# kohnakagawa/md_neighbor_list

Measured on AMD Instinct MI355X. Metric: Verlet-list build ms and Mpairs/s at N=1M rho=1.0; achieved HBM GB/s, higher is better.
Workload: dtype f32

## Files before the change

### md_neighbor_list_amd/csrc/nl_api.hip

```cpp
#include "../../include/nl_hip.h"

#include <hip/hip_runtime.h>

#include <algorithm>
#include <cmath>
#include <cstdio>
#include <cstdlib>
#include <cstring>
#include <new>
#include <tuple>
#include <type_traits>
#include <vector>

#include "nl_devbuf.hpp"
#include "nl_kernels.hpp"
#include "nl_stage.hpp"

using namespace nl;

namespace {

struct HostResult {
  uint32_t status;
  uint32_t tickets[17];
// ... 24 lines not shown
  auto tie() const { return std::tie(q, stride, gid, n_rows, n, n_ghost_lo, z_lo, mzl, slab, dyn, dyn_host, n_est); }
  bool operator==(const BuildArgs& o) const { return tie() == o.tie(); }
};

enum Binning : int32_t {
  BINNING_BUCKET,
  BINNING_TWO_PASS,
  BINNING_ATOMIC,
};
enum Search : int32_t {
  SEARCH_ROWS,
  SEARCH_MASKS,
  SEARCH_DENSE,
  SEARCH_SWEEPS,
};

struct BuildPlan {
  int32_t binning = BINNING_ATOMIC;
  int32_t cap_row = 0;
  bool split = false;
  int32_t search = SEARCH_SWEEPS;
  int32_t rows_v = 0;
  int32_t mask_nb = 1;
  bool small = false;
  bool rows12 = false;
  bool list = true;
  bool full = false;
  bool wide = false;
  bool filter = false;
  bool images = false;
  int32_t pbc = 0;
  int32_t idc = 0;
  int32_t id_shift = 0;
  bool id_rows = false;
  Box box = {{0, 0, 0}, 0, 0, 0};
  int32_t tilt = 0;
  auto tie() const {
    return std::tie(binning, cap_row, split, search, rows_v, mask_nb, small, rows12, list, full, wide, filter, images, pbc, idc, id_shift, id_rows,
                    box.L[0], box.L[1], box.L[2], box.xy, box.xz, box.yz, tilt);
  }
  bool operator==(const BuildPlan& o) const { return tie() == o.tie(); }
};

struct GraphKey {
  BuildArgs args;
  BuildPlan plan;
  int64_t capacity = 0;
  uint64_t buffers_epoch = 0;
  uint64_t ex_gen = 0;
  uint64_t ty_gen = 0;
  int32_t update = 0;
  double skin = 0;
  auto tie() const { return std::tie(args, plan, capacity, buffers_epoch, ex_gen, ty_gen, update, skin); }
  bool operator==(const GraphKey& o) const { return tie() == o.tie(); }
};

}

struct nl_handle_s {
  int dtype = NL_F32, device = 0;
  double rc = 0, L[3] = {0, 0, 0}, rc2 = 0;
  int32_t m[3] = {0, 0, 0};
  int64_t ncell = 0;
  double xy = 0, xz = 0, yz = 0, shear[3] = {0, 0, 0}, L0[3] = {0, 0, 0};
  int64_t mesh_cells_cap = 0, mesh_rows_cap = 0;
  DevBuf<double> lat_dev;
  float ims_f[3];
  double ims_d[3];
  float rc2_f = 0;
  float ms_f[3];

// ... 10 lines not shown
  DevBuf<int32_t> sorted_gid;
  DevBuf<int32_t> count;
  DevBuf<void> key_pointer;
  DevBuf<void> kp_alt;
  bool kp_alt_valid = false;
  int offset_width = 0;
  DevBuf<int32_t> progress;
  int32_t* row_count = nullptr;
  DevBuf<int32_t> row_start;
  DevBuf<int32_t> blk_base;
  DevBuf<void> tmp_pos;
  DevBuf<int32_t> tmp_row;
  size_t tmp_slots = 0;
  DevBuf<int32_t> row_cursor;
  int bucket_env = 1;
  int32_t bucket_scale = 1;
  bool bucket_off = false;
  int32_t bin_blocks = 0, bin_chunk = 0;
  bool bin_two_level = true;
  DevBuf<void> base_sorted;
  DevBuf<uint32_t> masks;
  DevBuf<int32_t> full27_list;
  DevBuf<void> resort_buf;
  int rows_env = -1;
  size_t dense_masks_limit = (size_t)64 << 30;
  int sweep_variant = 3;
  int num_cus = 256;
  DevBuf<unsigned long long> dbg_buf;
  int dbg_flags = 0;
  DevBuf<int32_t> cell_count;
  DevBuf<int32_t> cell_start;
  DevBuf<int32_t> cls_start;
  int idclass_env = 2;
  DevBuf<uint64_t> scan_look;
  int32_t scan_blocks = 0;
  DevBuf<int64_t> totals;
  uint32_t* status = nullptr;
  DevBuf<int32_t> list;
  DevBuf<int32_t> t_list;
  DevBuf<int32_t> t_count;
  DevBuf<int32_t> t_cursor;
  int64_t t_rows_cap = 0;
  int32_t t_max = 0;
  bool t_valid = false;

  HostResult* host = nullptr;
  hipStream_t own_stream = nullptr;
  bool use_graph = false;
  hipGraph_t graph = nullptr;
  hipGraphExec_t graph_exec = nullptr;
  GraphKey graph_key;
  uint64_t buffers_epoch = 1;
  bool begun = false;
  hipStream_t last_stream = nullptr;
  hipEvent_t ev[NL_NUM_STAGES + 1] = {};

  BuildArgs args;
  BuildPlan plan;
  int32_t list_quiet = 0;
  int64_t reruns[2] = {0, 0};
  bool built = false, pending = false;
  int32_t n = 0, n_rows = 0;
  int last_error = NL_OK, last_hip = 0;

  double skin = 0;
  const uint32_t* gate = nullptr;
// ... 286 lines not shown
template <typename T> SweepArgs<T> sweep_args(nl_handle_t h) {
  SweepArgs<T> a;
  a.sorted = static_cast<const Pos<T>*>(h->sorted);
  a.sorted_row = h->sorted_row;
  a.sorted_gid = h->plan.id_rows ? h->sorted_row : h->sorted_gid;
  a.cell_start = h->cell_start;
  a.cls_start = h->cls_start;
  a.mx = h->m[0], a.my = h->m[1], a.mzl = h->args.mzl, a.slab = h->args.slab;
  a.div_mx = fastdiv_make((uint32_t)h->m[0]), a.div_my = fastdiv_make((uint32_t)h->m[1]);
  a.rc2 = sizeof(T) == 4 ? (T)h->rc2_f : (T)h->rc2;
  a.count = h->count;
  a.progress = h->progress;
  a.key_pointer = search_kp(h);
  a.wide = h->plan.wide ? 1 : 0;
  a.n_rows = h->n_rows;
  a.list = search_list(h);
  a.total = h->totals + 1;
  a.capacity = h->capacity;
  a.status = h->status;
  a.masks = h->masks;
  a.masks_hi = reinterpret_cast<uint8_t*>(h->masks.get()) + h->masks.bytes() / MASK_ROW_BYTES * MASK_LO_BYTES;
  a.isplit = 1;
  a.mask_nb = h->plan.mask_nb;
  a.full27_list = h->full27_list;
  a.full27_count = reinterpret_cast<int32_t*>(h->status) + META_FULL27;
  a.fill_list_count = reinterpret_cast<int32_t*>(h->status) + META_FILL_LIST;
  a.pbc = h->plan.pbc;
  for (int d = 0; d < 3; d++) a.ms[d] = (T)(h->L[d] / h->m[d]);
  for (int d = 0; d < 3; d++) a.L[d] = (T)h->L[d];
  a.z_origin = h->args.slab ? h->args.z_lo - 1 : 0;
  a.dbg = h->dbg_flags;
  a.dbg_buf = h->dbg_buf;
  a.gate = h->gate;
  for (int d = 0; d < 3; d++) a.k[d] = (T)h->shear[d];
  a.lat = h->lat_dev;
  return a;
}

RowsArgs rows_args(nl_handle_t h) {
  RowsArgs a;
  a.sorted = static_cast<const Pos<float>*>(h->sorted);
  a.sorted_row = h->sorted_row, a.sorted_gid = h->plan.id_rows ? h->sorted_row : h->sorted_gid;
  a.fine_start = h->cell_start;
  a.mx = h->m[0], a.my = h->m[1], a.mzl = h->args.mzl, a.slab = h->args.slab;
  a.div_mx = fastdiv_make((uint32_t)h->m[0]), a.div_my = fastdiv_make((uint32_t)h->m[1]);
  a.rc2 = h->rc2_f;
  a.count = h->count;
  a.masks = h->masks;
  a.key_pointer = search_kp(h);
  a.list = search_list(h);
  a.total = h->totals + 1;
  a.capacity = h->capacity;
  a.status = h->status;
  a.over_list = h->full27_list;
  a.over_count = reinterpret_cast<int32_t*>(h->status) + META_FULL27;
  a.wide = h->plan.wide ? 1 : 0;
  a.dbg_buf = h->dbg_buf;
  a.gate = h->gate;
  return a;
}

template <int V, bool FULL, typename OFF> void launch_rows(nl_handle_t h, int mode, int32_t ncells, hipStream_t s) {
  const RowsArgs a = rows_args(h);
  const int32_t over_grid = 2 * h->num_cus;
  if (mode == MODE_COUNT) {
    hipLaunchKernelGGL((k_sweep_rows_f32<V, FULL>), dim3(ncells), dim3(ROWS_WAVES * WAVE), 0, s, a);
// ... 62 lines not shown
        count_masks();
        return;
      }
      if (h->n > 0)
        hipLaunchKernelGGL(k_row_base<OFF>, dim3((h->n + 255) / 256), dim3(256), 0, s, static_cast<const OFF*>(search_kp(h)),
                           h->sorted_row, h->n_rows, h->n, static_cast<OFF*>(h->base_sorted), h->gate);
      hipLaunchKernelGGL((k_fill_dense<T, FULL, PBC, OFF>), cells, dim3(FD_WAVES * WAVE), 0, s, a, static_cast<const OFF*>(h->base_sorted));
      return;
    default:
      if (mode == MODE_FILL) hipLaunchKernelGGL((k_sweep<T, MODE_FILL, FULL, PBC>), cells, wg, 0, s, a);
      else if constexpr (sizeof(T) == 4) hipLaunchKernelGGL((k_sweep_count_f32<FULL, PBC>), cells, wg, 0, s, a);
      else hipLaunchKernelGGL((k_sweep<T, MODE_COUNT, FULL, PBC>), cells, wg, 0, s, a);
  }
}

template <typename T, typename OFF> void launch_sweep_kind(nl_handle_t h, int mode, hipStream_t s) {
  const bool pbc = h->plan.pbc != 0;
  if (h->plan.full) pbc ? launch_search<T, true, true, OFF>(h, mode, s) : launch_search<T, true, false, OFF>(h, mode, s);
  else pbc ? launch_search<T, false, true, OFF>(h, mode, s) : launch_search<T, false, false, OFF>(h, mode, s);
}

template <typename T> void launch_sweep(nl_handle_t h, int mode, hipStream_t s) {
  if (h->plan.wide) launch_sweep_kind<T, int64_t>(h, mode, s);
  else launch_sweep_kind<T, int32_t>(h, mode, s);
}

bool mask_rows_ready(nl_handle_t h, int64_t nb, size_t row_bytes = MASK_ROW_BYTES) {
  const size_t need = row_bytes * (size_t)nb * ((size_t)h->n_max + 64);
  if (need > h->dense_masks_limit) return false;
  if (need > h->masks.bytes() || !h->masks) return dev_alloc(h, h->masks, need) == NL_OK;
  return true;
}

bool two_level_ok(nl_handle_t h, int32_t mzl) {
  return h->bin_two_level && (int64_t)h->m[1] * mzl <= BIN_MAX_ROWS && h->m[0] <= BIN_MAX_MX;
}

bool rows_layout_ok(nl_handle_t h, int32_t mzl) {
  const int64_t nrows = (int64_t)h->m[1] * mzl;
  return h->bin_two_level && nrows <= BIN_MAX_ROWS && h->m[0] <= BIN_FINE_MAX_MX && 4 * (int64_t)h->m[0] * nrows < 2147483000LL;
}
bool rows_margin_ok(nl_handle_t h) {
  const double ms = h->L[2] / h->m[2];
  return ms / h->rc >= 1.0 + 8.0 * h->m[2] * 5.9604644775390625e-8 + 9.5367431640625e-7;
}

template <typename T> int32_t bucket_cap(nl_handle_t h, int32_t n, int32_t mzl) {
  if (!h->bucket_env || h->bucket_off || !two_level_ok(h, mzl)) return 0;
  const int64_t nrows = (int64_t)h->m[1] * mzl;
  const int64_t cap = (int64_t)h->bucket_scale * ((int64_t)(1.25 * (double)n / (double)nrows) + 256);
  const size_t slots = (size_t)(nrows * cap) + 16;
  if (slots > 4 * ((size_t)h->n_max + 16) + 512 * (size_t)nrows) {
    h->bucket_off = true;
    return 0;
  }
  if (slots > h->tmp_slots) {
    if (dev_alloc(h, h->tmp_pos, sizeof(Pos<T>) * slots) || dev_alloc(h, h->tmp_row, sizeof(int32_t) * slots)) {
      h->bucket_off = true;
      h->tmp_slots = 0;
      const size_t n_slots = (size_t)h->n_max + 16;
      if (dev_alloc(h, h->tmp_pos, sizeof(Pos<T>) * n_slots) == NL_OK && dev_alloc(h, h->tmp_row, sizeof(int32_t) * n_slots) == NL_OK)
        h->tmp_slots = n_slots, h->last_error = NL_OK;
      return 0;
    }
    h->tmp_slots = slots;
  }
// ... 20 lines not shown
  if (sizeof(T) == 4 && variant3 && p.pbc == 0 && h->rows_env != 0 && rows_layout_ok(h, a.mzl) && rows_margin_ok(h)) {
    int v = -1;
    if (h->rows_env > 0 && h->rows_env <= 3) {
      v = h->rows_env - 1;
    } else if (h->rows_env == 4 || !sparse_enough) {
      const double span = mean_stream * 27.0 / 36.0;
      const int cap[3] = {RowsCfg<0>::CAP, RowsCfg<1>::CAP, RowsCfg<2>::CAP}, bits[3] = {16, 32, 32};
      for (int k = 0; k < 3 && v < 0; k++)
        if (mean_stream + 5.0 * std::sqrt(mean_stream) <= cap[k] && span + 6.0 * std::sqrt(span) <= 64.0 * bits[k]) v = k;
    }
    if (v >= 0 && mask_rows_ready(h, 1, v == 0 ? 128 : 256)) rows = true, p.rows_v = v, masks = true;
  }
  if (variant3 && !sparse_enough) {
    const int64_t nb = (int64_t)((mean_stream + 5.0 * std::sqrt(mean_stream) + 64.0) / SweepCfg<T>::CAP) + 1;
    if (nb <= FD_NB && mask_rows_ready(h, nb)) masks = true, p.mask_nb = (int32_t)nb;
  }
  p.search = rows ? SEARCH_ROWS : !masks ? SEARCH_SWEEPS : p.mask_nb > 1 ? SEARCH_DENSE : SEARCH_MASKS;
  p.small = sizeof(T) == 4 && p.search == SEARCH_MASKS && p.pbc == 0 &&
            mean_stream + 5.0 * std::sqrt(mean_stream) <= (double)LEAN_SMALL_CAP;
  p.rows12 = (double)a.n <= 21.0 * (double)std::max<int64_t>(1, ncl);

  const bool two_level = two_level_ok(h, a.mzl);
  p.split = part != PART_ALL && two_level && a.slab;
  const bool again_ok = !p.split && !a.dyn && !rerun;
  p.list = !again_ok || h->list_quiet < LIST_QUIET_BUILDS;
  p.cap_row = again_ok ? bucket_cap<T>(h, n, a.mzl) : 0;
  p.binning = !two_level ? BINNING_ATOMIC : p.cap_row > 0 ? BINNING_BUCKET : BINNING_TWO_PASS;
  p.id_rows = !a.gid && !p.tilt && p.binning != BINNING_ATOMIC;
  if (sizeof(T) == 4 && p.search == SEARCH_MASKS && !p.small && !p.full && p.pbc == 0 && h->idclass_env > 0 && !a.gid &&
      !a.slab && !a.dyn && !p.split && p.binning != BINNING_ATOMIC && h->m[0] * h->idclass_env <= 4 * BIN_FINE_MAX_MX &&
      h->m[0] >= 3 && h->m[1] >= 3 && a.mzl >= 3 && n > 0) {
    p.idc = h->idclass_env;
    while (((uint32_t)(n - 1) >> p.id_shift) >= (uint32_t)p.idc) p.id_shift++;
  }
  return p;
}

BuildPlan plan_for(nl_handle_t h, const BuildArgs& a, int part, bool rerun) {
  return h->dtype == NL_F32 ? plan_build<float>(h, a, part, rerun) : plan_build<double>(h, a, part, rerun);
}

void adopt_build(nl_handle_t h, const BuildArgs& a, const BuildPlan& p) {
  h->args = a;
  h->plan = p;
  h->ex_relabel = true;
  h->kp_alt_valid = false;
}

template <typename T, bool BUCKET, typename L> void launch_unrolled(nl_handle_t h, L&& launch) {
  auto by_id = [&](auto u) {
    if (h->plan.id_rows) launch(u, std::true_type());
    else launch(u, std::false_type());
  };
  if constexpr (sizeof(T) == 4 || !BUCKET) {
    if (h->bin_chunk >= 8 * BIN_THREADS) return by_id(std::integral_constant<int, 8>());
  }
  by_id(std::integral_constant<int, 4>());
}

template <typename T>
void launch_bin_cells(nl_handle_t h, const Grid<T>& g, int32_t grid, int32_t nrows, const int32_t* row_start, const BinPhase& ph,
                      int32_t cap_row, hipStream_t s) {
  auto launch_as = [&](auto fine, auto idc, auto idrow) {
    hipLaunchKernelGGL((k_bin_cells<T, decltype(fine)::value, decltype(idc)::value, decltype(idrow)::value>), dim3(grid), dim3(256), 0, s, g, nrows, row_start,
                       static_cast<const Pos<T>*>(h->tmp_pos), h->tmp_row, h->cell_start, static_cast<Pos<T>*>(h->sorted),
                       h->sorted_row, h->sorted_gid, ph, cap_row, h->cls_start, h->plan.id_shift);
// ... 386 lines not shown
  h->dtype = dtype, h->device = dev, h->rc = rc;
  h->rc2 = rc * rc;
  h->rc2_f = floor_to_float(h->rc2);
  for (int d = 0; d < 3; d++) {
    h->L[d] = L[d], h->m[d] = m[d], h->L0[d] = L[d];
    const float ms_f = (float)(L[d] / m[d]);
    h->ms_f[d] = ms_f;
    h->ims_f[d] = (float)(1.0 / (double)ms_f);
    const double ms_d = L[d] / m[d];
    h->ims_d[d] = 1.0 / ms_d;
  }
  h->ncell = (int64_t)m[0] * m[1] * m[2];
  double lat0[LATTICE_CODES * 3];
  lattice_table(box_of(h), lat0);
  if (h->lat_dev.replace(sizeof(lat0)) != hipSuccess ||
      hipMemcpy(h->lat_dev, lat0, sizeof(lat0), hipMemcpyHostToDevice) != hipSuccess ||
      hipStreamCreateWithFlags(&h->own_stream, hipStreamNonBlocking) != hipSuccess ||
      hipHostMalloc(reinterpret_cast<void**>(&h->host), sizeof(HostResult), hipHostMallocDefault) != hipSuccess) {
    nl_destroy(h);
    return NL_ERR_HIP;
  }
  for (auto& e : h->ev)
    if (hipEventCreate(&e) != hipSuccess) {
      nl_destroy(h);
      return NL_ERR_HIP;
    }
  memset(h->host, 0, sizeof(HostResult));
  {
    hipDeviceProp_t prop;
    if (hipGetDeviceProperties(&prop, dev) == hipSuccess && prop.multiProcessorCount > 0) h->num_cus = prop.multiProcessorCount;
    if (const char* v = getenv("NL_SWEEP_VARIANT")) h->sweep_variant = atoi(v) <= 1 ? 1 : 3;
    if (const char* v = getenv("NL_ROWS")) h->rows_env = std::max(-1, std::min(atoi(v), 4));
    if (const char* v = getenv("NL_IDCLASS")) h->idclass_env = atoi(v) >= 4 ? 4 : atoi(v) >= 2 ? 2 : 0;
    if (const char* v = getenv("NL_OFFSET_WIDTH")) h->offset_width = atoi(v) == 64 ? 64 : atoi(v) == 32 ? 32 : 0;
    if (const char* v = getenv("NL_BINNING")) h->bin_two_level = atoi(v) != 1;
    if (const char* v = getenv("NL_BIN_BUCKETS")) h->bucket_env = atoi(v) != 0;
    if (const char* v = getenv("NL_GRAPH")) h->use_graph = atoi(v) != 0;
    if (const char* v = getenv("NL_DEBUG_FLAGS")) h->dbg_flags = atoi(v);
  }
  *out = h;
  return NL_OK;
}

int nl_destroy(nl_handle_t h) {
  if (!h) return NL_ERR_ARG;
  (void)hipSetDevice(h->device);
  if (h->pending && h->last_stream) (void)hipStreamSynchronize(h->last_stream);
  if (h->host) (void)hipHostFree(h->host);
  for (auto& e : h->ev)
    if (e) (void)hipEventDestroy(e);
  if (h->graph_exec) (void)hipGraphExecDestroy(h->graph_exec);
  if (h->graph) (void)hipGraphDestroy(h->graph);
  if (h->own_stream) (void)hipStreamDestroy(h->own_stream);
  delete h;
  return NL_OK;
}

int nl_initialize(nl_handle_t h, int32_t n_max) {
  if (!h || n_max < 0) return fail(h, NL_ERR_ARG);
  HIPCHK(h, hipSetDevice(h->device));
  if (h->pending) {
    int rc = finish(h, false);
    (void)rc;
  }
  h->built = false;
  h->upd_valid = false;
// ... 435 lines not shown
  HIPCHK(h, hipDeviceSynchronize());
  HIPCHK(h, hipMemcpy(out, h->dbg_buf, 8 * (size_t)n, hipMemcpyDeviceToHost));
  if (reset) HIPCHK(h, hipMemset(h->dbg_buf, 0, 8 * (64 + 4 * 4096)));
  return NL_OK;
}

int nl_debug_occupancy(int32_t out[8]) {
  if (!out) return NL_ERR_ARG;
  int v = 0;
  hipDeviceProp_t prop;
  if (hipGetDeviceProperties(&prop, 0) != hipSuccess) return NL_ERR_NO_DEVICE;
  out[0] = (int32_t)(prop.maxSharedMemoryPerMultiProcessor / 1024);
  out[1] = (int32_t)(prop.sharedMemPerBlock / 1024);
  out[2] = out[3] = 0;
  (void)hipOccupancyMaxActiveBlocksPerMultiprocessor(&v, k_sweep_count_f32<false, false>, SWEEP_WAVES * WAVE, 0);
  out[4] = v;
  (void)hipOccupancyMaxActiveBlocksPerMultiprocessor(&v, k_sweep<float, MODE_FILL>, SWEEP_WAVES * WAVE, 0);
  out[5] = v;
  hipFuncAttributes fa;
  (void)hipFuncGetAttributes(&fa, reinterpret_cast<const void*>(k_sweep_count_masks_f32<false, false>));
  out[6] = (int32_t)fa.sharedSizeBytes;
  out[7] = fa.numRegs;
  return NL_OK;
}

int nl_get_build_info(nl_handle_t h, int32_t info[8]) {
  if (!h || !info) return NL_ERR_ARG;
  for (int k = 4; k < 8; k++) info[k] = 0;
  const BuildPlan& p = h->plan;
  info[4] = p.wide ? 64 : 32;
  info[5] = p.mask_nb;
  info[6] = p.search == SEARCH_ROWS ? 1 + p.rows_v : 0;
  const int32_t binning = p.binning == BINNING_TWO_PASS ? 0 : p.binning == BINNING_BUCKET ? 1 : 2;
  info[7] = (p.small ? 1 : 0) | p.idc << 8 | binning << 16;
  info[0] = p.search != SEARCH_SWEEPS ? 1 : 0;
  info[1] = h->sweep_variant;
  info[2] = h->dtype == NL_F32 ? SweepCfg<float>::CAP : SweepCfg<double>::CAP;
  info[3] = h->num_cus;
  return NL_OK;
}

int nl_get_build_stats(nl_handle_t h, int64_t stats[4]) {
  if (!h || !stats) return NL_ERR_ARG;
  stats[0] = h->reruns[0];
  stats[1] = h->reruns[1];
  stats[2] = h->plan.cap_row;
  stats[3] = h->plan.list ? 1 : 0;
  return NL_OK;
}

int nl_last_error(nl_handle_t h) { return h ? h->last_error : NL_ERR_ARG; }
int nl_last_hip_error(nl_handle_t h) { return h ? h->last_hip : 0; }

int nl_profile_last_build(nl_handle_t h, int32_t reps, double ms[NL_NUM_STAGES]) {
  if (!h || !ms || reps <= 0) return fail(h, NL_ERR_ARG);
  int rc = nl_synchronize(h);
  if (rc) return rc;
  HIPCHK(h, hipSetDevice(h->device));
  for (int k = 0; k < NL_NUM_STAGES; k++) ms[k] = 0;
  hipStream_t s = h->own_stream;
  HIPCHK(h, hipStreamSynchronize(h->last_stream));
  BuildArgs a = h->args;
  a.n = h->n;
  const BuildPlan p = plan_for(h, a, PART_ALL, false);
  for (int r = 0; r < reps; r++) {
    rc = dispatch_build(h, a, p, s, h->ev);
    if (rc) return rc;
// ... 86 lines not shown
```

### md_neighbor_list_amd/csrc/nl_kernels.hpp

```cpp
#pragma once

#include <hip/hip_runtime.h>
#include <stdint.h>

#include <type_traits>

namespace nl {

constexpr int WAVE = 64;

enum : uint32_t { ST_OUT_OF_BOX = 1u, ST_CAPACITY = 2u, ST_DOMAIN = 4u, ST_INDEX_OVERFLOW = 8u, ST_ROW_OVERFLOW = 16u, ST_ID_RANGE = 32u };

template <typename T> struct Pos;
template <> struct alignas(16) Pos<float> {
  float x, y, z;
  int32_t gid;
};
template <> struct alignas(32) Pos<double> {
  double x, y, z;
  int32_t gid;
  int32_t row;
};

struct Box {
// ... 778 lines not shown
  const Pos<T>* __restrict__ sorted;
  const int32_t* __restrict__ sorted_row;
  const int32_t* __restrict__ sorted_gid;
  const int32_t* __restrict__ cell_start;
  const int32_t* __restrict__ cls_start;
  int32_t mx, my, mzl, slab;
  FastDiv div_mx, div_my;
  T rc2;
  int32_t* __restrict__ count;
  int32_t* __restrict__ progress;
  const void* __restrict__ key_pointer;
  int32_t wide;
  int32_t n_rows;
  int32_t* __restrict__ list;
  const int64_t* __restrict__ total;
  int64_t capacity;
  uint32_t* __restrict__ status;
  T L[3];
  int32_t pbc;
  T ms[3];
  int32_t z_origin;
  int32_t isplit;
  int32_t mask_nb;
  int32_t* __restrict__ full27_list;
  int32_t* __restrict__ full27_count;
  int32_t* __restrict__ fill_list_count;
  uint32_t* __restrict__ masks;
  uint8_t* __restrict__ masks_hi;
  unsigned long long* dbg_buf;
  int32_t dbg;
  const uint32_t* gate = nullptr;
  T k[3];
  const double* lat;
};

template <typename T>
__device__ __forceinline__ void face_shift(const SweepArgs<T>& a, int32_t wr, T& sx, T& sy, T& sz) {
  T s[3];
  lattice_shift(a.lat, wr, s);
  sx = s[0], sy = s[1], sz = s[2];
}

__device__ __forceinline__ void recheck_image(const SweepArgs<double>& a, int32_t wr, Pos<double>& pe) {
  const double* p = a.lat + 3 * wr;
  pe.x = add_rn(pe.x, p[0]);
  __builtin_amdgcn_sched_barrier(0);
  pe.y = add_rn(pe.y, p[1]);
  __builtin_amdgcn_sched_barrier(0);
  pe.z = add_rn(pe.z, p[2]);
}

template <typename T> struct SweepCfg;
constexpr int MASK_LO_BYTES = 2 * WAVE, MASK_HI_BYTES = WAVE, MASK_ROW_BYTES = MASK_LO_BYTES + MASK_HI_BYTES;
__device__ __forceinline__ bool hi_plane_used(int32_t mask_nb, int32_t ntiles) { return mask_nb > 1 || ntiles > 16; }
template <bool NT = false>
__device__ __forceinline__ void mask_store(uint32_t* masks, uint8_t* masks_hi, size_t row, int lane, uint32_t bits, bool hi) {
  uint16_t* const lo_p = reinterpret_cast<uint16_t*>(reinterpret_cast<char*>(masks) + row * MASK_LO_BYTES) + lane;
  uint8_t* const hi_p = masks_hi + row * MASK_HI_BYTES + lane;
  if constexpr (NT) {
    __builtin_nontemporal_store((uint16_t)bits, lo_p);
    if (hi) __builtin_nontemporal_store((uint8_t)(bits >> 16), hi_p);
  } else {
    *lo_p = (uint16_t)bits;
    if (hi) *hi_p = (uint8_t)(bits >> 16);
  }
}
// ... 704 lines not shown
  }
  c.total_j = carry;
  return true;
}
template <int IDC> __device__ __forceinline__ bool cls_setup(const SweepArgs<float>& a, int lane, ClsCtx<IDC>& c) {
  const int32_t w = xcd_cell_index();
  const int32_t wy = (int32_t)fastdiv((uint32_t)w, a.div_mx), cx = w - wy * a.mx;
  const int32_t cz = (int32_t)fastdiv((uint32_t)wy, a.div_my), cy = wy - cz * a.my;
  return cls_setup_at(a, lane, cx, cy, cz, c);
}

template <int IDC, int NW, typename E>
__device__ __forceinline__ void cls_stage(const E* __restrict__ from, const ClsCtx<IDC>& c, E* dst, int lane, int wave) {
#pragma unroll 1
  for (int32_t pc = wave; pc < 9 * IDC; pc += NW) {
    const int32_t w = 3 * pc;
    const int32_t s0 = c.get(c.src, w), l0 = c.get(c.len, w), s1 = c.get(c.src, w + 1), l1 = c.get(c.len, w + 1);
    const int32_t s2 = c.get(c.src, w + 2), l2 = c.get(c.len, w + 2), off = c.get(c.off, w);
    const int32_t len = l0 + l1 + l2;
#pragma unroll 1
    for (int32_t kb = 0; kb < len; kb += WAVE) {
      const int32_t i = kb + lane;
      if (i < len) {
        const int32_t at = i < l0 ? s0 + i : i < l0 + l1 ? s1 + (i - l0) : s2 + (i - l0 - l1);
        const __attribute__((address_space(1))) void* const gp = (const __attribute__((address_space(1))) void*)(from + at);
        __attribute__((address_space(3))) void* const lp = (__attribute__((address_space(3))) void*)(dst + off + kb);
        if constexpr (sizeof(E) == 16) __builtin_amdgcn_global_load_lds(gp, lp, 16, 0, 0);
        else __builtin_amdgcn_global_load_lds(gp, lp, 4, 0, 0);
      }
    }
  }
}

template <bool FULL> constexpr int EXPAND_RMAX_OF = FULL ? 192 : 160;
constexpr int EXPAND_WAVES = 2;

template <typename T, bool FULL = false, bool PBC = false, typename OFF = int32_t, int RB = 24, int EW = EXPAND_WAVES, int CAP = SweepCfg<T>::CAP,
          int IDC = 0>
__global__ void __launch_bounds__(EW* WAVE, (sizeof(OFF) == 8 ? 4 : sizeof(T) == 4 ? (FULL || RB > 12 ? 7 : 8) : 4)) __attribute__((amdgpu_num_sgpr(80)))
k_fill_masks(SweepArgs<T> a) {
  static_assert(IDC == 0 || (sizeof(T) == 4 && !FULL && !PBC), "id classes: fp32 half list, open box");
  if (gate_closed(a.gate)) return;
  constexpr int EXPAND_RMAX = EXPAND_RMAX_OF<FULL>;
  __shared__ __attribute__((aligned(32))) int32_t lds[CAP + EW * 4 * EXPAND_RMAX];
  int32_t* const gids = lds;
  const int tid = threadIdx.x, lane = tid & 63, wave = __builtin_amdgcn_readfirstlane(tid >> 6);
#if NL_STAMP_FILL
  uint64_t ft_prev = __builtin_amdgcn_s_memtime(), ft_acc[6] = {0, 0, 0, 0, 0, 0};
  auto fstamp = [&](int phase) {
    const uint64_t now = __builtin_amdgcn_s_memtime();
    ft_acc[phase] += now - ft_prev;
    ft_prev = now;
  };
#endif
  const int64_t total = a.total[0];
  typename std::conditional<(IDC > 0), ClsCtx<IDC ? IDC : 2>, CellCtx>::type c;
  bool ok;
  if constexpr (IDC > 0) ok = cls_setup<IDC>(a, lane, c);
  else ok = cell_setup(a, lane, c);
#if NL_STAMP_FILL
  fstamp(0);
#endif
  if (total > a.capacity) {
    if (blockIdx.x == 0 && threadIdx.x == 0) atomicOr(a.status, ST_CAPACITY);
    return;
  }
  if (!ok) return;
  if (c.total_j > CAP) {
    if (tid == 0) a.full27_list[atomicAdd(a.fill_list_count, 1)] = c.cx + (c.cy + c.cz * a.my) * a.mx;
    return;
  }

  const int32_t per_wave = (c.ni + EW - 1) / EW;
  const int32_t r_beg = min(wave * per_wave, c.ni), r_end = min(r_beg + per_wave, c.ni);
  uint32_t w[RB];
  OFF base_l;
  const bool hi_plane = hi_plane_used(1, (c.total_j + WAVE - 1) / WAVE);
  auto load_rows = [&](int32_t r0) {
    {
      const int32_t srow = a.sorted_row[c.ibeg + r0 + min(lane, RB - 1)];
      base_l = static_cast<const OFF*>(a.key_pointer)[min((uint32_t)srow, (uint32_t)a.n_rows)];
    }
    const size_t slot0 = (size_t)(c.ibeg + r0);
    const char* const lo0 = reinterpret_cast<const char*>(a.masks) + slot0 * MASK_LO_BYTES;
    if (hi_plane) {
      const uint8_t* const hi0 = a.masks_hi + slot0 * MASK_HI_BYTES;
#pragma unroll
      for (int u = 0; u < RB; u++)
        w[u] = (uint32_t)mask_ld<EW == 2>(reinterpret_cast<const uint16_t*>(lo0 + u * MASK_LO_BYTES) + lane) | (uint32_t)mask_ld<EW == 2>(hi0 + u * MASK_HI_BYTES + lane) << 16;
    } else {
#pragma unroll
      for (int u = 0; u < RB; u++) w[u] = (uint32_t)mask_ld<EW == 2>(reinterpret_cast<const uint16_t*>(lo0 + u * MASK_LO_BYTES) + lane);
    }
  };
  auto base = [&](int u) -> OFF {
    const uint32_t lo = (uint32_t)__builtin_amdgcn_readlane((int32_t)(uint32_t)base_l, u);
    if constexpr (sizeof(OFF) == 4) return (OFF)lo;
    const uint32_t hi = (uint32_t)__builtin_amdgcn_readlane((int32_t)(uint32_t)((uint64_t)base_l >> 32), u);
    return (OFF)((uint64_t)hi << 32 | lo);
  };
  load_rows(r_beg);
  if (a.dbg & 32) return;

  int32_t cls_row[IDC > 0 ? IDC : 1], cls_t0[IDC > 0 ? IDC : 1];
  if constexpr (IDC > 0) {
#pragma unroll
    for (int k = 0; k < IDC; k++) {
      cls_row[k] = c.get(c.src, 27 * k + CLS_OWN) - c.ibeg;
      cls_t0[k] = c.get(c.off, 27 * k) & ~(WAVE - 1);
    }
    cls_stage<IDC, EW>(a.sorted_gid, c, gids, lane, wave);
  } else
#pragma unroll
  for (int s = 0; s < (NSEG + EW - 1) / EW; s++) {
    const int sg = min(wave + s * EW, NSEG - 1);
    const int32_t len = wave + s * EW < NSEG ? __builtin_amdgcn_readlane(c.seg_len, sg) : 0;
    const int32_t src = __builtin_amdgcn_readlane(c.seg_src, sg);
    const int32_t off = __builtin_amdgcn_readlane(c.seg_off, sg);
    for (int32_t kb = 0; kb < len; kb += WAVE) {
      if (kb + lane < len)
        __builtin_amdgcn_global_load_lds((const __attribute__((address_space(1))) void*)(a.sorted_gid + src + kb + lane),
                                         (__attribute__((address_space(3))) void*)(gids + off + kb), 4, 0, 0);
    }
  }
#if NL_STAMP_FILL
  fstamp(1);
#endif
  __syncthreads();
#if NL_STAMP_FILL
  fstamp(2);
#endif

  const int32_t* const g = gids + lane;
  for (int32_t r0 = r_beg; r0 < r_end; r0 += RB) {
    if (r0 != r_beg) load_rows(r0);
#pragma unroll
    for (int u0 = 0; u0 < RB; u0 += 4) {
      if (r0 + u0 >= r_end) continue;
      uint32_t word[4], ptr[4];
      int32_t nrow[4];
      const int32_t* gq[4];
#pragma unroll
      for (int q = 0; q < 4; q++) {
        if constexpr (IDC > 0) {
          int32_t t0 = cls_t0[0];
#pragma unroll
          for (int k = 1; k < IDC; k++) t0 = r0 + u0 + q >= cls_row[k] ? cls_t0[k] : t0;
          gq[q] = g + t0;
        } else {
          gq[q] = g;
        }
      }
#pragma unroll
      for (int q = 0; q < 4; q++) {
        word[q] = r0 + u0 + q < r_end ? (w[u0 + q] & 0xFFFFFFu) : 0u;
        if (a.dbg & 16) word[q] = 0;
        const int32_t cnt = __popc(word[q]);
        const int32_t incl = scan64_dpp(cnt);
        nrow[q] = __builtin_amdgcn_readlane(incl, 63);
        ptr[q] = (uint32_t)(incl - cnt);
      }
      const int32_t nmax = max(max(nrow[0], nrow[1]), max(nrow[2], nrow[3]));
#if NL_STAMP_FILL
      fstamp(3);
// ... 230 lines not shown
```

### md_neighbor_list_amd/csrc/nl_lean.hpp

```cpp
#pragma once

namespace nl {

constexpr int PIPE_G = 7;

template <int NW = SWEEP_WAVES>
__device__ __forceinline__ void pipe_stage(const SweepArgs<float>& a, const CellCtx& c, Pos<float>* dst, int tid, int lane, int wave) {
#pragma unroll 1
  for (int sg = wave; sg < NSEG; sg += NW) {
    const int32_t len = __builtin_amdgcn_readlane(c.seg_len, sg);
    const int32_t src = __builtin_amdgcn_readlane(c.seg_src, sg);
    const int32_t off = __builtin_amdgcn_readlane(c.seg_off, sg);
#pragma unroll 1
    for (int32_t kb = 0; kb < len; kb += WAVE) {
      if (kb + lane < len)
        __builtin_amdgcn_global_load_lds((const __attribute__((address_space(1))) void*)(a.sorted + src + kb + lane),
                                         (__attribute__((address_space(3))) void*)(dst + off + kb), 16, 0, 0);
    }
  }
  const int32_t pad = c.total_j + tid;
  if (pad < ((c.total_j + WAVE - 1) & ~(WAVE - 1))) {
    Pos<float> sentinel;
    sentinel.x = 1.0e18f, sentinel.y = 0.f, sentinel.z = 0.f, sentinel.gid = INT32_MIN;
    dst[pad] = sentinel;
// ... 190 lines not shown
        case 1: class_pipe_group<1>(a, tile, t0, tsplit, ntiles, lane, pi_l, p); break;
        case 2: class_pipe_group<2>(a, tile, t0, tsplit, ntiles, lane, pi_l, p); break;
        case 3: class_pipe_group<3>(a, tile, t0, tsplit, ntiles, lane, pi_l, p); break;
        case 4: class_pipe_group<4>(a, tile, t0, tsplit, ntiles, lane, pi_l, p); break;
        case 5: class_pipe_group<5>(a, tile, t0, tsplit, ntiles, lane, pi_l, p); break;
        case 6: class_pipe_group<6>(a, tile, t0, tsplit, ntiles, lane, pi_l, p); break;
        default: class_pipe_group<7>(a, tile, t0, tsplit, ntiles, lane, pi_l, p); break;
      }
      p.row_l = row_l, p.slot0 = slot_b + i0, p.gcount = gcount;
    }
  }
}

template <int IDC, int NW = SWEEP_WAVES, int CAP = SweepCfg<float>::CAP>
__global__ void __launch_bounds__(NW* WAVE, 8) __attribute__((amdgpu_num_sgpr(80))) k_sweep_class_f32(SweepArgs<float> a) {
  if (gate_closed(a.gate)) return;
  __shared__ __attribute__((aligned(32))) Pos<float> buf[CAP];
  const int tid = threadIdx.x, lane = tid & 63, wave = __builtin_amdgcn_readfirstlane(tid >> 6);
  __builtin_amdgcn_s_setprio(NL_PRIO);
  ClsCtx<IDC> c;
  if (!cls_setup<IDC>(a, lane, c)) return;
  if (c.total_j > CAP) {
    if (tid == 0) a.full27_list[atomicAdd(a.full27_count, 1)] = c.cx + (c.cy + c.cz * a.my) * a.mx;
    return;
  }
  cls_stage<IDC, NW>(a.sorted, c, buf, lane, wave);
  const int32_t pad = c.total_j + tid;
  if (pad < ((c.total_j + WAVE - 1) & ~(WAVE - 1))) {
    Pos<float> sentinel;
    sentinel.x = 1.0e18f, sentinel.y = 0.f, sentinel.z = 0.f, sentinel.gid = INT32_MIN;
    buf[pad] = sentinel;
  }
  asm volatile("s_waitcnt vmcnt(0) lgkmcnt(0)\n\ts_barrier" ::: "memory");
  PipePending pend;
  pend.gcount = 0, pend.mine = 0, pend.row_l = 0, pend.slot0 = 0;
  class_search<IDC, NW>(a, c, buf, lane, wave, pend);
  pipe_flush<NW == SWEEP_WAVES>(a, pend, lane, hi_plane_used(1, (c.total_j + WAVE - 1) / WAVE));
}

template <bool FULL>
__global__ void __launch_bounds__(SWEEP_WAVES* WAVE) __attribute__((amdgpu_num_sgpr(80))) k_sweep_list_f32(SweepArgs<float> a) {
  if (gate_closed(a.gate)) return;
  constexpr int CAP = SweepCfg<float>::CAP;
  __shared__ __attribute__((aligned(32))) Pos<float> tile[CAP];
  const int tid = threadIdx.x, lane = tid & 63, wave = __builtin_amdgcn_readfirstlane(tid >> 6);
  const int32_t count = *a.full27_count;
  for (int32_t idx = blockIdx.x; idx < count; idx += gridDim.x) {
    if (idx != (int32_t)blockIdx.x) __syncthreads();
    const int32_t cell = a.full27_list[idx];
    const int32_t row = cell / a.mx, cx = cell - row * a.mx, cz = row / a.my, cy = row - cz * a.my;
    CellCtx c;
    if (!cell_setup_at(a, lane, cx, cy, cz, c)) continue;
    cell_search<float, MODE_COUNT_MASKS, CAP, SWEEP_WAVES, FULL, false, false>(a, c, tile, tid, lane, wave);
  }
}

}
```

### md_neighbor_list_amd/neighlist.py

```python
from __future__ import annotations

import ctypes as C

import torch

from . import _lib
from ._lib import NLError, check


class _DevView:

    def __init__(self, ptr, shape, typestr, owner):
        self.__cuda_array_interface__ = {
            "shape": tuple(int(s) for s in shape),
            "typestr": typestr,
            "data": (int(ptr), False),
            "version": 2,
            "strides": None,
        }
        self._owner = owner


def _as_tensor(ptr, shape, typestr, owner, device):
    n = 1
# ... 527 lines not shown
        ptr, n = C.c_void_p(), C.c_int32()
        check(self._lib.nl_get_cell_order(self._h, C.byref(ptr), C.byref(n)), "nl_get_cell_order")
        return _as_tensor(ptr.value, (n.value,), "<i4", self, self.device)

    def resort(self, *arrays):
        stream = torch.cuda.current_stream(self.device).cuda_stream
        for t in arrays:
            if not isinstance(t, torch.Tensor) or t.device.type != "cuda" or not t.is_contiguous() or t.shape[0] != self._n:
                raise TypeError("resort() takes contiguous device tensors with one leading entry per particle")
            check(self._lib.nl_resort(self._h, t.data_ptr(), t.element_size() * (t.numel() // max(t.shape[0], 1)), stream), "nl_resort")

    def sorted_state(self):
        cs, sp, sr, ncl = C.c_void_p(), C.c_void_p(), C.c_void_p(), C.c_int64()
        check(self._lib.nl_get_sorted(self._h, C.byref(cs), C.byref(sp), C.byref(sr), C.byref(ncl)), "nl_get_sorted")
        entries = ncl.value * (4 if self.build_info()["fine_rows"] else 1) + 1
        return (_as_tensor(cs.value, (entries,), "<i4", self, self.device),
                _as_tensor(sr.value, (self._n,), "<i4", self, self.device))

    def profile_stages(self, q, reps=10):
        n = self._check_q(q, None)
        ms = (C.c_double * _lib.NL_NUM_STAGES)()
        check(self._lib.nl_profile_stages(self._h, q.data_ptr(), q.shape[1], n, int(reps), C.byref(ms)),
              "nl_profile_stages")
        self._n = self._n_rows = n
        return dict(zip(_lib.STAGE_NAMES, (float(v) for v in ms)))


    def build_info(self):
        info = (C.c_int32 * 8)()
        check(self._lib.nl_get_build_info(self._h, C.byref(info)), "nl_get_build_info")
        return {"masks": bool(info[0]), "variant": int(info[1]), "lds_batch": int(info[2]), "cus": int(info[3]),
                "offset_bits": int(info[4]), "mask_rows": int(info[5]), "fine_rows": int(info[6]),
                "small_cells": int(info[7]) & 0xFF, "id_classes": int(info[7]) >> 8 & 0xFF,
                "binning": ("two_pass", "bucket", "atomic")[int(info[7]) >> 16 & 3]}

    def build_stats(self):
        st = (C.c_int64 * 4)()
        check(self._lib.nl_get_build_stats(self._h, C.byref(st)), "nl_get_build_stats")
        return {"row_overflow_reruns": int(st[0]), "list_reruns": int(st[1]), "cap_row": int(st[2]),
                "list_launched": bool(st[3])}

    def profile_last_build(self, reps=10):
        ms = (C.c_double * _lib.NL_NUM_STAGES)()
        check(self._lib.nl_profile_last_build(self._h, int(reps), C.byref(ms)), "nl_profile_last_build")
        return dict(zip(_lib.STAGE_NAMES, (float(v) for v in ms)))


def axes_mask(axes) -> int:
    if isinstance(axes, str):
        if any(c not in "xyz" for c in axes.lower()):
            raise ValueError(f"periodic axes {axes!r}: use letters from 'xyz'")
        return sum(1 << "xyz".index(c) for c in set(axes.lower()))
    if not hasattr(axes, "__len__"):
        return 7 if axes else 0
    axes = tuple(axes)
    if len(axes) != 3:
        raise ValueError(f"periodic axes {axes!r}: a 3-tuple of bools or a string from 'xyz'")
    return sum(1 << d for d in range(3) if axes[d])


def npairs_exceeds_int32(nl) -> bool:
    n = C.c_int64()
    check(nl._lib.nl_number_of_pairs(nl._h, C.byref(n)), "nl_number_of_pairs")
    return (2 if nl.full_list else 1) * int(n.value) > 2147483647


def device_count() -> int:
# ... 4 lines not shown
```

Measured before the change: 167,900.

## Cull staged neighbor atoms outside the cell bounding-box reach before class search

Adds a per-cell culling pass to the id-class mask search. It computes the bounding box of the cell's own atoms with a wave-wide min reduction, then drops staged neighbor atoms whose distance to that box exceeds the cutoff (plus a small margin). Survivors are compacted in LDS and the kept-bit words are saved per cell so the list-expansion kernel can remap offsets and staged ids the same way. This is meant to cut pair tests in the search and fill stages. The cost is an extra reduction, two barriers, a compaction pass and a global bitmask buffer per cell.

```diff
diff --git a/md_neighbor_list_amd/csrc/nl_api.hip b/md_neighbor_list_amd/csrc/nl_api.hip
--- a/md_neighbor_list_amd/csrc/nl_api.hip
+++ b/md_neighbor_list_amd/csrc/nl_api.hip
@@ -80,11 +80,12 @@
   int32_t pbc = 0;
   int32_t idc = 0;
   int32_t id_shift = 0;
+  bool cull = false;
   bool id_rows = false;
   Box box = {{0, 0, 0}, 0, 0, 0};
   int32_t tilt = 0;
   auto tie() const {
-    return std::tie(binning, cap_row, split, search, rows_v, mask_nb, small, rows12, list, full, wide, filter, images, pbc, idc, id_shift, id_rows,
+    return std::tie(binning, cap_row, split, search, rows_v, mask_nb, small, rows12, list, full, wide, filter, images, pbc, idc, id_shift, cull, id_rows,
                     box.L[0], box.L[1], box.L[2], box.xy, box.xz, box.yz, tilt);
   }
   bool operator==(const BuildPlan& o) const { return tie() == o.tie(); }
@@ -161,6 +162,8 @@
   DevBuf<int32_t> cell_start;
   DevBuf<int32_t> cls_start;
   int idclass_env = 2;
+  DevBuf<uint64_t> cull_bits;
+  int cull_env = 1;
   DevBuf<uint64_t> scan_look;
   int32_t scan_blocks = 0;
   DevBuf<int64_t> totals;
@@ -513,6 +516,7 @@
   a.dbg = h->dbg_flags;
   a.dbg_buf = h->dbg_buf;
   a.gate = h->gate;
+  a.cull_bits = h->plan.cull ? h->cull_bits.get() : nullptr;
   for (int d = 0; d < 3; d++) a.k[d] = (T)h->shear[d];
   a.lat = h->lat_dev;
   return a;
@@ -641,6 +645,10 @@
   return true;
 }
 
+bool cull_bits_ready(nl_handle_t h, int64_t cells) {
+  return follow(h, h->cull_bits, cells, sizeof(uint64_t) * CULL_WORDS * (size_t)cells) == NL_OK;
+}
+
 bool two_level_ok(nl_handle_t h, int32_t mzl) {
   return h->bin_two_level && (int64_t)h->m[1] * mzl <= BIN_MAX_ROWS && h->m[0] <= BIN_MAX_MX;
 }
@@ -727,6 +735,7 @@
       h->m[0] >= 3 && h->m[1] >= 3 && a.mzl >= 3 && n > 0) {
     p.idc = h->idclass_env;
     while (((uint32_t)(n - 1) >> p.id_shift) >= (uint32_t)p.idc) p.id_shift++;
+    p.cull = h->cull_env != 0 && cull_bits_ready(h, ncl);
   }
   return p;
 }
@@ -1179,6 +1188,7 @@
     if (const char* v = getenv("NL_SWEEP_VARIANT")) h->sweep_variant = atoi(v) <= 1 ? 1 : 3;
     if (const char* v = getenv("NL_ROWS")) h->rows_env = std::max(-1, std::min(atoi(v), 4));
     if (const char* v = getenv("NL_IDCLASS")) h->idclass_env = atoi(v) >= 4 ? 4 : atoi(v) >= 2 ? 2 : 0;
+    if (const char* v = getenv("NL_CULL")) h->cull_env = atoi(v) != 0;
     if (const char* v = getenv("NL_OFFSET_WIDTH")) h->offset_width = atoi(v) == 64 ? 64 : atoi(v) == 32 ? 32 : 0;
     if (const char* v = getenv("NL_BINNING")) h->bin_two_level = atoi(v) != 1;
     if (const char* v = getenv("NL_BIN_BUCKETS")) h->bucket_env = atoi(v) != 0;
@@ -1680,7 +1690,7 @@
   info[5] = p.mask_nb;
   info[6] = p.search == SEARCH_ROWS ? 1 + p.rows_v : 0;
   const int32_t binning = p.binning == BINNING_TWO_PASS ? 0 : p.binning == BINNING_BUCKET ? 1 : 2;
-  info[7] = (p.small ? 1 : 0) | p.idc << 8 | binning << 16;
+  info[7] = (p.small ? 1 : 0) | p.idc << 8 | binning << 16 | (p.cull ? 1 : 0) << 18;
   info[0] = p.search != SEARCH_SWEEPS ? 1 : 0;
   info[1] = h->sweep_variant;
   info[2] = h->dtype == NL_F32 ? SweepCfg<float>::CAP : SweepCfg<double>::CAP;
diff --git a/md_neighbor_list_amd/csrc/nl_kernels.hpp b/md_neighbor_list_amd/csrc/nl_kernels.hpp
--- a/md_neighbor_list_amd/csrc/nl_kernels.hpp
+++ b/md_neighbor_list_amd/csrc/nl_kernels.hpp
@@ -834,6 +834,7 @@
   const uint32_t* gate = nullptr;
   T k[3];
   const double* lat;
+  uint64_t* cull_bits = nullptr;
 };
 
 template <typename T>
@@ -1604,6 +1605,124 @@
   }
 }
 
+constexpr int CULL_WORDS = SweepCfg<float>::CAP / WAVE;
+constexpr float CULL_DELTA = 1.0f / (float)(1 << 20);
+
+__device__ __forceinline__ float min_raw(float a, float b) {
+  float r;
+  asm("v_min_f32 %0, %1, %2" : "=v"(r) : "v"(a), "v"(b));
+  return r;
+}
+__device__ __forceinline__ void wave_min6(float (&v)[6]) {
+#define NL_MIN6_STEP(ctrl) \
+  "v_min_f32_dpp %0, %0, %0 " ctrl "\n\tv_min_f32_dpp %1, %1, %1 " ctrl "\n\tv_min_f32_dpp %2, %2, %2 " ctrl "\n\t" \
+  "v_min_f32_dpp %3, %3, %3 " ctrl "\n\tv_min_f32_dpp %4, %4, %4 " ctrl "\n\tv_min_f32_dpp %5, %5, %5 " ctrl "\n\t"
+  asm("s_nop 1\n\t" NL_MIN6_STEP("row_shr:1 row_mask:0xf bank_mask:0xf") NL_MIN6_STEP("row_shr:2 row_mask:0xf bank_mask:0xf")
+      NL_MIN6_STEP("row_shr:4 row_mask:0xf bank_mask:0xf") NL_MIN6_STEP("row_shr:8 row_mask:0xf bank_mask:0xf")
+      NL_MIN6_STEP("row_bcast:15 row_mask:0xa bank_mask:0xf") NL_MIN6_STEP("row_bcast:31 row_mask:0xc bank_mask:0xf") "s_nop 1"
+      : "+v"(v[0]), "+v"(v[1]), "+v"(v[2]), "+v"(v[3]), "+v"(v[4]), "+v"(v[5]));
+#undef NL_MIN6_STEP
+#pragma unroll
+  for (int k = 0; k < 6; k++) v[k] = __builtin_bit_cast(float, __builtin_amdgcn_readlane(__builtin_bit_cast(int32_t, v[k]), 63));
+}
+
+struct CullMap {
+  uint32_t lo, hi;
+  int32_t excl;
+  int32_t kept;
+};
+__device__ __forceinline__ CullMap cull_map(uint64_t word) {
+  CullMap m;
+  m.lo = (uint32_t)word, m.hi = (uint32_t)(word >> 32);
+  const int32_t cnt = __popc(m.lo) + __popc(m.hi);
+  const int32_t incl = scan64_dpp(cnt);
+  m.excl = incl - cnt;
+  m.kept = __builtin_amdgcn_readlane(incl, 63);
+  return m;
+}
+__device__ __forceinline__ int32_t cull_rank(const CullMap& m, int32_t s) {
+  const int32_t at = (s >> 6) << 2, b = s & 63;
+  const uint32_t lo = (uint32_t)__builtin_amdgcn_ds_bpermute(at, (int32_t)m.lo), hi = (uint32_t)__builtin_amdgcn_ds_bpermute(at, (int32_t)m.hi);
+  const int32_t ex = __builtin_amdgcn_ds_bpermute(at, m.excl);
+  const uint32_t below_lo = b >= 32 ? 0xFFFFFFFFu : (1u << (b & 31)) - 1u, below_hi = b > 32 ? (1u << (b & 31)) - 1u : 0u;
+  return ex + __popc(lo & below_lo) + __popc(hi & below_hi);
+}
+__device__ __forceinline__ bool cull_slot(const CullMap& m, int32_t t, int32_t& dst) {
+  const uint32_t lo = (uint32_t)__builtin_amdgcn_readlane((int32_t)m.lo, t), hi = (uint32_t)__builtin_amdgcn_readlane((int32_t)m.hi, t);
+  dst = __builtin_amdgcn_readlane(m.excl, t) + (int32_t)__builtin_amdgcn_mbcnt_hi(hi, __builtin_amdgcn_mbcnt_lo(lo, 0u));
+  return (((uint64_t)hi << 32 | lo) >> (threadIdx.x & 63) & 1u) != 0;
+}
+template <int IDC> __device__ __forceinline__ void cull_offsets(const CullMap& m, ClsCtx<IDC>& c) {
+#pragma unroll
+  for (int j = 0; j < ClsCtx<IDC>::NT; j++) c.off[j] = cull_rank(m, c.off[j]);
+  c.total_j = m.kept;
+}
+
+template <int IDC, int NW, int CAP>
+__device__ __forceinline__ void cls_cull(const SweepArgs<float>& a, ClsCtx<IDC>& c, Pos<float>* buf, int32_t cell, int tid, int lane, int wave) {
+  constexpr int TW = (CAP / WAVE + NW - 1) / NW;
+  static_assert(CAP / WAVE == CULL_WORDS && CAP % WAVE == 0, "a ballot word per tile of the buffer");
+  const int32_t nj = c.total_j, ntiles = (nj + WAVE - 1) / WAVE;
+  uint64_t* const out = a.cull_bits + (size_t)cell * CULL_WORDS;
+  if (ntiles * WAVE > CAP - WAVE) {
+    if (wave == 0 && lane < ntiles) out[lane] = lane + 1 < ntiles ? ~0ull : ~0ull >> (ntiles * WAVE - nj);
+    return;
+  }
+  uint64_t* const words = reinterpret_cast<uint64_t*>(buf + CAP) - CULL_WORDS;
+  const float inf = __builtin_inff();
+  float bx[6] = {inf, inf, inf, inf, inf, inf};
+  float chk = 0.f;
+  for (int32_t kb = 0; kb < c.ni; kb += WAVE) {
+    int32_t i = min(kb + lane, c.ni - 1), slot = 0;
+#pragma unroll
+    for (int k = IDC - 1; k >= 0; k--) {
+      const int32_t own = c.get(c.off, 27 * k + CLS_OWN), first = c.get(c.src, 27 * k + CLS_OWN) - c.ibeg;
+      slot = (k == IDC - 1 || i < first + c.get(c.len, 27 * k + CLS_OWN)) ? own + (i - first) : slot;
+    }
+    const Pos<float> p = buf[slot];
+    bx[0] = min_raw(bx[0], p.x), bx[1] = min_raw(bx[1], p.y), bx[2] = min_raw(bx[2], p.z);
+    bx[3] = min_raw(bx[3], -p.x), bx[4] = min_raw(bx[4], -p.y), bx[5] = min_raw(bx[5], -p.z);
+    chk = chk + ((p.x + p.y) + p.z);
+  }
+  wave_min6(bx);
+  const float lx = bx[0], ly = bx[1], lz = bx[2], hx = -bx[3], hy = -bx[4], hz = -bx[5];
+  const float reach = __builtin_amdgcn_ballot_w64(chk != chk) != 0 ? inf : mul_rn(a.rc2, 1.0f + CULL_DELTA);
+  Pos<float> p[TW];
+#pragma unroll
+  for (int u = 0; u < TW; u++) p[u] = buf[min(wave + u * NW, ntiles - 1) * WAVE + lane];
+#pragma unroll
+  for (int u = 0; u < TW; u++) {
+    const int32_t t = wave + u * NW;
+    if (t >= ntiles) break;
+    const float gx = fmaxf(fmaxf(sub_rn(p[u].x, hx), sub_rn(lx, p[u].x)), 0.f);
+    const float gy = fmaxf(fmaxf(sub_rn(p[u].y, hy), sub_rn(ly, p[u].y)), 0.f);
+    const float gz = fmaxf(fmaxf(sub_rn(p[u].z, hz), sub_rn(lz, p[u].z)), 0.f);
+    float g2 = add_rn(add_rn(mul_rn(gx, gx), mul_rn(gy, gy)), mul_rn(gz, gz));
+    g2 = __builtin_fmaf(add_rn(add_rn(p[u].x, p[u].y), p[u].z), 0.f, g2);
+    uint64_t kept = __builtin_amdgcn_ballot_w64(!(g2 > reach));
+    if (t == ntiles - 1) kept &= ~0ull >> (ntiles * WAVE - nj);
+    if (lane == 0) words[t] = kept;
+  }
+  asm volatile("s_waitcnt lgkmcnt(0)\n\ts_barrier" ::: "memory");
+  const CullMap m = cull_map(lane < ntiles ? words[lane] : 0ull);
+  if (wave == 0 && lane < ntiles) out[lane] = (uint64_t)m.hi << 32 | m.lo;
+#pragma unroll
+  for (int u = 0; u < TW; u++) {
+    const int32_t t = wave + u * NW;
+    if (t >= ntiles) break;
+    int32_t dst;
+    if (cull_slot(m, t, dst)) buf[dst] = p[u];
+  }
+  const int32_t pad = m.kept + tid;
+  if (pad < ((m.kept + WAVE - 1) & ~(WAVE - 1))) {
+    Pos<float> sentinel;
+    sentinel.x = 1.0e18f, sentinel.y = 0.f, sentinel.z = 0.f, sentinel.gid = INT32_MIN;
+    buf[pad] = sentinel;
+  }
+  cull_offsets<IDC>(m, c);
+  asm volatile("s_waitcnt lgkmcnt(0)\n\ts_barrier" ::: "memory");
+}
+
 template <bool FULL> constexpr int EXPAND_RMAX_OF = FULL ? 192 : 160;
 constexpr int EXPAND_WAVES = 2;
 
@@ -1626,6 +1745,11 @@
   };
 #endif
   const int64_t total = a.total[0];
+  uint64_t kept_word = 0;
+  if constexpr (IDC > 0) {
+    static_assert(EW * 4 * EXPAND_RMAX >= CAP, "the staged ids of a cull build land in the row buffers");
+    if (a.cull_bits) kept_word = a.cull_bits[(size_t)xcd_cell_index() * CULL_WORDS + min(lane, CULL_WORDS - 1)];
+  }
   typename std::conditional<(IDC > 0), ClsCtx<IDC ? IDC : 2>, CellCtx>::type c;
   bool ok;
   if constexpr (IDC > 0) ok = cls_setup<IDC>(a, lane, c);
@@ -1647,7 +1771,14 @@
   const int32_t r_beg = min(wave * per_wave, c.ni), r_end = min(r_beg + per_wave, c.ni);
   uint32_t w[RB];
   OFF base_l;
-  const bool hi_plane = hi_plane_used(1, (c.total_j + WAVE - 1) / WAVE);
+  CullMap cm = {0u, 0u, 0, 0};
+  bool cull = false;
+  const int32_t staged_tiles = (c.total_j + WAVE - 1) / WAVE;
+  if constexpr (IDC > 0) {
+    cull = a.cull_bits != nullptr;
+    if (cull) cm = cull_map(lane < staged_tiles ? kept_word : 0ull);
+  }
+  const bool hi_plane = hi_plane_used(1, ((cull ? cm.kept : c.total_j) + WAVE - 1) / WAVE);
   auto load_rows = [&](int32_t r0) {
     {
       const int32_t srow = a.sorted_row[c.ibeg + r0 + min(lane, RB - 1)];
@@ -1675,13 +1806,10 @@
   if (a.dbg & 32) return;
 
   int32_t cls_row[IDC > 0 ? IDC : 1], cls_t0[IDC > 0 ? IDC : 1];
+  int32_t* const staged = cull ? lds + CAP : gids;
+  (void)staged;
   if constexpr (IDC > 0) {
-#pragma unroll
-    for (int k = 0; k < IDC; k++) {
-      cls_row[k] = c.get(c.src, 27 * k + CLS_OWN) - c.ibeg;
-      cls_t0[k] = c.get(c.off, 27 * k) & ~(WAVE - 1);
-    }
-    cls_stage<IDC, EW>(a.sorted_gid, c, gids, lane, wave);
+    cls_stage<IDC, EW>(a.sorted_gid, c, staged, lane, wave);
   } else
 #pragma unroll
   for (int s = 0; s < (NSEG + EW - 1) / EW; s++) {
@@ -1702,6 +1830,22 @@
 #if NL_STAMP_FILL
   fstamp(2);
 #endif
+  if constexpr (IDC > 0) {
+    if (cull) {
+      for (int32_t t = wave; t < staged_tiles; t += EW) {
+        int32_t dst;
+        const int32_t id = staged[t * WAVE + lane];
+        if (cull_slot(cm, t, dst)) gids[dst] = id;
+      }
+      cull_offsets<IDC>(cm, c);
+      __syncthreads();
+    }
+#pragma unroll
+    for (int k = 0; k < IDC; k++) {
+      cls_row[k] = c.get(c.src, 27 * k + CLS_OWN) - c.ibeg;
+      cls_t0[k] = c.get(c.off, 27 * k) & ~(WAVE - 1);
+    }
+  }
 
   const int32_t* const g = gids + lane;
   for (int32_t r0 = r_beg; r0 < r_end; r0 += RB) {
diff --git a/md_neighbor_list_amd/csrc/nl_lean.hpp b/md_neighbor_list_amd/csrc/nl_lean.hpp
--- a/md_neighbor_list_amd/csrc/nl_lean.hpp
+++ b/md_neighbor_list_amd/csrc/nl_lean.hpp
@@ -246,6 +246,7 @@
     buf[pad] = sentinel;
   }
   asm volatile("s_waitcnt vmcnt(0) lgkmcnt(0)\n\ts_barrier" ::: "memory");
+  if (a.cull_bits) cls_cull<IDC, NW, CAP>(a, c, buf, c.cx + (c.cy + c.cz * a.my) * a.mx, tid, lane, wave);
   PipePending pend;
   pend.gcount = 0, pend.mine = 0, pend.row_l = 0, pend.slot0 = 0;
   class_search<IDC, NW>(a, c, buf, lane, wave, pend);
diff --git a/md_neighbor_list_amd/neighlist.py b/md_neighbor_list_amd/neighlist.py
--- a/md_neighbor_list_amd/neighlist.py
+++ b/md_neighbor_list_amd/neighlist.py
@@ -583,7 +583,8 @@
         return {"masks": bool(info[0]), "variant": int(info[1]), "lds_batch": int(info[2]), "cus": int(info[3]),
                 "offset_bits": int(info[4]), "mask_rows": int(info[5]), "fine_rows": int(info[6]),
                 "small_cells": int(info[7]) & 0xFF, "id_classes": int(info[7]) >> 8 & 0xFF,
-                "binning": ("two_pass", "bucket", "atomic")[int(info[7]) >> 16 & 3]}
+                "binning": ("two_pass", "bucket", "atomic")[int(info[7]) >> 16 & 3],
+                "reach_cull": bool(int(info[7]) >> 18 & 1)}
 
     def build_stats(self):
         st = (C.c_int64 * 4)()
```

Result: faster. 177,400, median of 6 (+5.6%).
